# koadman/mauveAligner

Hardware: AMD Instinct MI355X
Metric: aligned Mbp/s (seed+extend+DP) (higher is better)
Workload: dtype u32

## Files before the change

mauvealigner_amd/csrc/chain_dev.hip:

```cpp
#include "common.hpp"
#include "dev_scan.hpp"
#include <cstring>
#include <cstdlib>

namespace {

using namespace devscan;
constexpr int CH_TILE = devscan::TILE;

constexpr int CH_CNT_ALIVE = 8, CH_CNT_CL = CH_CNT_ALIVE + MAUVE_MAX_SEQ, CH_CNT_WORDS = 128;
static_assert(CH_CNT_CL + MAUVE_MAX_SEQ <= CH_CNT_WORDS && CH_CNT_WORDS <= 256, "counter block");

struct ChKeyDst { uint32_t *key, *val, *key0, *val0; };
__device__ __forceinline__ void ch_put_key(const ChKeyDst &kd, uint32_t n, uint32_t i, int g, int32_t s, bool alive, uint32_t dead_key)
{
    uint32_t *k = g ? kd.key + (size_t)g * n : kd.key0, *v = g ? kd.val + (size_t)g * n : kd.val0;
    k[i] = alive ? (uint32_t)(s < 0 ? -s : s) : dead_key;
    v[i] = i;
}

__global__ void __launch_bounds__(256) ch_init(const int64_t *__restrict__ rlen, const int64_t *__restrict__ rst, uint32_t n, int N,
                                               int32_t *__restrict__ len, int32_t *__restrict__ st, uint32_t *__restrict__ crop,
                                               uint32_t *__restrict__ cnt, unsigned long long *__restrict__ weight, ChKeyDst kd, uint32_t dead_key)
{
// ... 116 lines not shown
    __device__ void total(uint32_t na, int y) const { if (y == 0) cnt[0] = na; }
};
struct LcbNodes {
    const int32_t *len, *st; uint32_t n; int N; const uint32_t *ordc, *rank; uint32_t *cnt; int32_t *node_of;
    unsigned long long *weight; uint32_t *orient; const uint32_t *gapid;
    const int64_t *mw;
    __device__ uint32_t domain(int) const { return cnt[0]; }
    __device__ bool flag(uint32_t k, int) const
    {
        if (k == 0) return true;
        const uint32_t i = ordc[k], p = ordc[k - 1];
        if (gapid && gapid[i] != gapid[p]) return true;
        bool brk = false;
#pragma unroll 4
        for (int g = 1; g < N; g++) {
            const bool oi = st[(size_t)i * N + g] < 0, op = st[(size_t)p * N + g] < 0;
            const uint32_t ri = rank[(size_t)g * n + i], rp = rank[(size_t)g * n + p];
            brk |= (oi != op) | (!oi ? ri != rp + 1 : ri + 1 != rp);
        }
        return brk;
    }
    __device__ void each(uint32_t k, uint32_t o, bool fl, int) const
    {
        const uint32_t i = ordc[k], nd = o + (fl ? 1u : 0u) - 1u;
        node_of[i] = (int32_t)nd;
        atomicAdd(&weight[nd], mw ? (unsigned long long)mw[i] : (unsigned long long)len[i] * (unsigned long long)N);
    }
    __device__ void emit(uint32_t k, uint32_t o, int) const
    {
        const uint32_t i = ordc[k];
        uint32_t ob = 0;
        for (int g = 0; g < N; g++) if (st[(size_t)i * N + g] < 0) ob |= 1u << g;
        orient[o] = ob;
    }
    __device__ void total(uint32_t K, int) const { cnt[1] = K; }
};
struct NodeSeq {
    uint32_t n; const uint32_t *ordc; uint32_t *cnt; const int32_t *node_of; int32_t *seq;
    __device__ uint32_t domain(int) const { return cnt[0]; }
    __device__ bool flag(uint32_t r, int y) const { return r == 0 || node_of[ordc[(size_t)y * n + r]] != node_of[ordc[(size_t)y * n + r - 1]]; }
    __device__ void each(uint32_t, uint32_t, bool, int) const {}
    __device__ void emit(uint32_t r, uint32_t o, int y) const { if (o < cnt[1]) seq[(size_t)y * cnt[1] + o] = node_of[ordc[(size_t)y * n + r]]; }
    __device__ void total(uint32_t t, int) const { if (t != cnt[1]) atomicAdd(&cnt[2], 1u); }
};
__global__ void __launch_bounds__(256) ch_links(int N, const uint32_t *__restrict__ cnt, const int32_t *__restrict__ seq,
                                                int32_t *__restrict__ prevv, int32_t *__restrict__ nextv)
{
    const uint32_t K = cnt[1], j = blockIdx.x * 256u + threadIdx.x;
    const int g = blockIdx.y;
// ... 85 lines not shown
        return;
    }
    uint32_t L[CH_CL_MAX], Ln[CH_CL_MAX], I[CH_CL_MAX], CF[CH_CL_MAX], CL[CH_CL_MAX], pf[CH_CL_MAX], pl[CH_CL_MAX];
    uint8_t F[CH_CL_MAX];
    ch_cluster_run(len, st, N, g, dead_key, eleft, eidx, a, s, L, Ln, I, CF, CL, pf, pl, F);
}

__global__ void __launch_bounds__(64) ch_cluster_pass_big(int32_t *__restrict__ len, int32_t *__restrict__ st, int N, int g, uint32_t dead_key,
                                                          uint32_t *__restrict__ eleft, uint32_t *__restrict__ eidx,
                                                          const uint32_t *__restrict__ cstart, const uint32_t *__restrict__ cnt_in,
                                                          uint32_t *__restrict__ ws, uint32_t n, int cl_max, uint32_t *__restrict__ fail, int big_max)
{
    const uint32_t j = blockIdx.x * 64u + threadIdx.x;
    if (j >= cnt_in[0]) return;
    const uint32_t a = cstart[j];
    const int s = (int)(cstart[j + 1] - a);
    if (s <= cl_max) return;
    if (s > big_max) { *fail = 1; return; }
    uint32_t *L = ws + a, *Ln = L + n, *I = Ln + n, *CF = I + n, *CL = CF + n, *pf = CL + n, *pl = pf + n;
    uint8_t *F = reinterpret_cast<uint8_t *>(ws + 7 * (size_t)n) + a;
    ch_cluster_run(len, st, N, g, dead_key, eleft, eidx, a, s, L, Ln, I, CF, CL, pf, pl, F);
}

__global__ void __launch_bounds__(256) ch_pack_graph(uint32_t K, int N, const unsigned long long *__restrict__ weight, const uint32_t *__restrict__ orient,
                                                     const int32_t *__restrict__ prevv, const int32_t *__restrict__ nextv, const uint32_t *__restrict__ cnt,
                                                     unsigned long long *__restrict__ out)
{
    const uint32_t i = blockIdx.x * 256u + threadIdx.x;
    uint32_t *o32 = reinterpret_cast<uint32_t *>(out + K);
    int32_t *op = reinterpret_cast<int32_t *>(o32 + K), *on = op + (size_t)K * N;
    if (i < K) { out[i] = weight[i]; o32[i] = orient[i]; }
    if (i < K * (uint32_t)N) { op[i] = prevv[i]; on[i] = nextv[i]; }
    if (i == 0) reinterpret_cast<uint32_t *>(on + (size_t)K * N)[0] = cnt[2];
}

__global__ void __launch_bounds__(256) ch_label(const int32_t *__restrict__ len, uint32_t n, const int32_t *__restrict__ node_of,
                                                const int32_t *__restrict__ final_id, int32_t *__restrict__ lcb)
{
    const uint32_t i = blockIdx.x * 256u + threadIdx.x;
    if (i >= n) return;
    lcb[i] = len[i] > 0 ? final_id[node_of[i]] : -1;
}

__global__ void __launch_bounds__(256) co_keys(const int32_t *__restrict__ lcb, const uint32_t *__restrict__ ord0, const uint32_t *__restrict__ cnt, uint32_t n, uint32_t nl,
                                               uint32_t *__restrict__ key, uint32_t *__restrict__ val, unsigned long long *__restrict__ lw, uint32_t *__restrict__ out)
{
    const uint32_t k = blockIdx.x * 256u + threadIdx.x;
    if (k < nl) lw[k] = 0;
    if (k < 2) out[k] = 0;
    if (k >= n) return;
    if (k < cnt[0]) {
// ... 117 lines not shown
        for (int j = lane; j < kk; j += 64) {
            int v = j;
            while (!s_alive[v] && s_merged[v] >= 0) v = s_merged[v];
            node_ok[n0 + j] = s_alive[v] ? 1 : 0;
        }
    }
}
struct GapSurvivors {
    const int32_t *len, *st, *node_of; const uint32_t *gapid; const uint8_t *node_ok; uint32_t n; int N;
    int32_t *olen, *ost; uint32_t *ogap; uint32_t *total_out;
    __device__ uint32_t domain(int) const { return n; }
    __device__ bool flag(uint32_t i, int) const { return len[i] > 0 && node_ok[node_of[i]]; }
    __device__ void each(uint32_t, uint32_t, bool, int) const {}
    __device__ void emit(uint32_t i, uint32_t o, int) const
    {
        olen[o] = len[i]; ogap[o] = gapid[i];
        for (int g = 0; g < N; g++) ost[(size_t)o * N + g] = st[(size_t)i * N + g];
    }
    __device__ void total(uint32_t t, int) const { *total_out = t; }
};

}

int chain_order_device(mauve_ctx *c, int N, int64_t nl, int64_t min_gap, int64_t *na_out, int64_t *n_rec_out)
{
    const uint32_t n = (uint32_t)c->dev_rec_n;
    *na_out = 0; *n_rec_out = 0;
    if (nl <= 0) return MAUVE_OK;
    const int32_t *len = c->ch_len.as<int32_t>(), *lcb = len + 2 * (size_t)n;
    const int32_t *st = c->ch_st.as<int32_t>();
    uint32_t *k1 = c->ch_ent.as<uint32_t>(), *v1 = k1 + n, *k2 = v1 + n, *v2 = k2 + n;
    HIPCHK(c, c->ch_anch.ensure((size_t)n * (2 + (size_t)N) * 4 + 64));
    HIPCHK(c, c->ch_lw.ensure((size_t)nl * 8 + 64));
    int32_t *alen = c->ch_anch.as<int32_t>(), *ast = alen + n, *alcb = ast + (size_t)n * N;
    unsigned long long *lw = c->ch_lw.as<unsigned long long>();
    uint32_t *cnt = c->ch_cnt.as<uint32_t>();
    const uint32_t blocks = (n + 255) / 256;
    int bits = 1; while ((1LL << bits) <= nl) bits++;
    hipLaunchKernelGGL(co_keys, dim3(blocks), dim3(256), 0, c->stream, lcb, c->ch_ord.as<uint32_t>() + (size_t)n * N , cnt, n, (uint32_t)nl, k1, v1, lw, cnt + 16);
    uint32_t *kk = k1, *vv = v1;
    int rc = sort_pairs_u32(c, n, bits, &kk, &vv, k2, v2, MAUVE_K_MISC);
    if (rc) return rc;
    hipLaunchKernelGGL(co_gather, dim3(blocks), dim3(256), 0, c->stream, kk, vv, n, (uint32_t)nl, N, len, st, min_gap, alen, ast, alcb, lw, cnt + 16);
    HIPCHK(c, hipGetLastError());
    HIPCHK(c, c->pin_chain.ensure(256));
    HIPCHK(c, hipMemcpyAsync(c->pin_chain.p, cnt + 16, 8, hipMemcpyDeviceToHost, c->stream));
    HIPCHK(c, hipStreamSynchronize(c->stream));
    *na_out = c->pin_chain.as<uint32_t>()[0];
    *n_rec_out = c->pin_chain.as<uint32_t>()[1];
    return MAUVE_OK;
}

struct ChSpGenomes { uint64_t word_off[MAUVE_MAX_SEQ]; int32_t s[4][4]; };
template <int MODE>
__global__ void __launch_bounds__(256) ch_sp_scores(const uint64_t *__restrict__ packed, ChSpGenomes G, int N, const int32_t *__restrict__ len, const int32_t *__restrict__ st,
                                                    uint32_t n, int64_t *__restrict__ out, SpMult M)
{
    const int lane = threadIdx.x & 63;
    const uint32_t wave = (blockIdx.x * 256u + threadIdx.x) >> 6, nw = (gridDim.x * 256u) >> 6;
    for (uint32_t i = wave; i < n; i += nw) {
        const int64_t L = len[i];
        int64_t acc = 0;
        for (int64_t c = lane; c < L; c += 64) {
            uint32_t have = 0, bases = 0;
            uint64_t mlo = 0, mhi = 0;
            for (int g = 0; g < N; g++) {
                const int64_t s0 = st[(size_t)i * N + g];
// ... 34 lines not shown
    HIPCHK(c, c->ch_st.ensure((size_t)n * N * 4));
    HIPCHK(c, c->ch_crop.ensure((size_t)n * 8));
    const uint32_t nb = (n + CH_TILE - 1) / CH_TILE;
    const size_t sl_words = ((size_t)N * ((size_t)n + 1) + 15) & ~(size_t)15, flag_bytes = ((size_t)N * n + 63) & ~(size_t)63;
    HIPCHK(c, c->ch_ent.ensure((size_t)n * 4 * 4 + sl_words * 4 + flag_bytes + (size_t)nb * 4 * 3 * (size_t)N + 64));
    HIPCHK(c, c->ch_ord.ensure((size_t)n * N * 4 * 3));
    HIPCHK(c, c->ch_rank.ensure((size_t)n * N * 4));
    HIPCHK(c, c->ch_cnt.ensure((size_t)CH_CNT_WORDS * 4));
    if (seg0) HIPCHK(c, c->ch_big.ensure((size_t)n * 29 + 64));
    int32_t *len = c->ch_len.as<int32_t>(), *node_of = len + n;
    uint32_t *gapid = seg0 ? reinterpret_cast<uint32_t *>(len + 3 * (size_t)n) : nullptr;
    int32_t *st = c->ch_st.as<int32_t>();
    uint32_t *crop = c->ch_crop.as<uint32_t>();
    uint32_t *sl = c->ch_ent.as<uint32_t>() + 4 * (size_t)n;
    uint8_t *cflag = reinterpret_cast<uint8_t *>(sl + sl_words);
    uint32_t *bmax = reinterpret_cast<uint32_t *>(cflag + flag_bytes), *balive = bmax + (size_t)N * nb, *bcnt = balive + (size_t)N * nb;
    uint32_t *ord = c->ch_ord.as<uint32_t>(), *ordc = ord + (size_t)n * N, *okey = ordc + (size_t)n * N;
    uint32_t *rank = c->ch_rank.as<uint32_t>();
    uint32_t *cnt = c->ch_cnt.as<uint32_t>();
    const int64_t *rlen = c->sorted_rec.as<int64_t>(), *rst = rlen + n;
    const uint32_t blocks = (n + 255) / 256;
    const int big_max = switches().ch_big_max;
    const int cl_set = switches().ch_cl_max, cl_max = cl_set && cl_set < CH_CL_MAX ? cl_set : CH_CL_MAX;
    HIPCHK(c, c->ch_graph.ensure((size_t)n * (8 + 4 + (size_t)N * 4 * 3 + 4) + 8 + (size_t)n * (8 + 4 + (size_t)N * 8) + 64));
    unsigned long long *weight = c->ch_graph.as<unsigned long long>();
    const int sort_passes = (pos_bits + 1 + 7) / 8;
    const bool odd = sort_passes & 1;
    const int g_lo = seg0 ? 0 : 1;
    const ChKeyDst kd{odd ? rank : okey, odd ? ordc : ord, seg0 && odd ? rank : okey, seg0 && odd ? ordc : ord};
    if (seg0) hipLaunchKernelGGL(ch_init_seg, dim3(blocks), dim3(256), 0, c->stream, rlen, rst, n, N, seg0, nseg, len, st, crop, gapid, cnt, weight, kd, dead_key);
    else hipLaunchKernelGGL(ch_init, dim3(blocks), dim3(256), 0, c->stream, rlen, rst, n, N, len, st, crop, cnt, weight, kd, dead_key);
    if (g_lo < N) {
        uint32_t *kk = kd.key + (size_t)g_lo * n, *vv = kd.val + (size_t)g_lo * n;
        int rc = sort_pairs_u32_batch(c, (uint32_t)(N - g_lo), n, n, pos_bits + 1, &kk, &vv, (odd ? okey : rank) + (size_t)g_lo * n,
                                      (odd ? ord : ordc) + (size_t)g_lo * n, MAUVE_K_MISC);
        if (rc) return rc;
        if (kk != okey + (size_t)g_lo * n || vv != ord + (size_t)g_lo * n) { c->err = "chain_device: the orders did not land in place"; return MAUVE_ERR_STATE; }
    }
    hipLaunchKernelGGL(cl_partial, dim3(nb, N), dim3(256), 0, c->stream, len, n, dead_key, okey, ord, bmax, balive);
    hipLaunchKernelGGL(cl_flags, dim3(nb, N), dim3(256), 0, c->stream, len, n, dead_key, okey, ord, bmax, balive, nb, cflag, cnt, bcnt);
    const ClusterStarts cs{cflag, n, sl, cnt};
    hipLaunchKernelGGL((cmp_write<ClusterStarts>), dim3(nb, N), dim3(256), 0, c->stream, cs, bcnt);
    for (int g = 0; g < N; g++) {
        uint32_t *og = ord + (size_t)g * n, *kg = okey + (size_t)g * n, *sg = sl + (size_t)g * ((size_t)n + 1);
        hipLaunchKernelGGL(ch_cluster_pass, dim3(blocks), dim3(256), 0, c->stream, len, st, N, g, dead_key, kg, og, sg, cnt + CH_CNT_CL + g, cnt + 3, seg0 ? 1 : 0, cl_max);
        if (seg0) hipLaunchKernelGGL(ch_cluster_pass_big, dim3((n + 63) / 64), dim3(64), 0, c->stream, len, st, N, g, dead_key, kg, og, sg, cnt + CH_CNT_CL + g,
                                     c->ch_big.as<uint32_t>(), n, cl_max, cnt + 3, big_max);
// ... 13 lines not shown
        memcpy(SG.s, sp_scoring->matrix, sizeof SG.s);
        SpMult M; memset(&M, 0, sizeof M);
        if (c->rp_now != MAUVE_REPEAT_PENALTY_OFF) {
            if (c->rp_gen != c->genome_gen) { c->err = "chain_device: repeat multiplicities missing"; return MAUVE_ERR_STATE; }
            M.p = c->rp_mult.as<uint8_t>();
            for (int g = 0; g < N; g++) M.off[g] = c->rp_off[(size_t)g];
        }
        const dim3 grid((uint32_t)std::min<size_t>(((size_t)n + 3) / 4, 256 * 8));
        if (c->rp_now == MAUVE_REPEAT_PENALTY_NEGATIVE)
            hipLaunchKernelGGL(ch_sp_scores<MAUVE_REPEAT_PENALTY_NEGATIVE>, grid, dim3(256), 0, c->stream, c->genomes.as<uint64_t>(), SG, N, len, st, n, c->ch_mw.as<int64_t>(), M);
        else if (c->rp_now == MAUVE_REPEAT_PENALTY_ZERO)
            hipLaunchKernelGGL(ch_sp_scores<MAUVE_REPEAT_PENALTY_ZERO>, grid, dim3(256), 0, c->stream, c->genomes.as<uint64_t>(), SG, N, len, st, n, c->ch_mw.as<int64_t>(), M);
        else
            hipLaunchKernelGGL(ch_sp_scores<MAUVE_REPEAT_PENALTY_OFF>, grid, dim3(256), 0, c->stream, c->genomes.as<uint64_t>(), SG, N, len, st, n, c->ch_mw.as<int64_t>(), M);
        mw = c->ch_mw.as<int64_t>();
    }
    const LcbNodes ln{len, st, n, N, ordc, rank, cnt, node_of, weight, orient, gapid, mw};
    hipLaunchKernelGGL((cmp_count<LcbNodes>), dim3(nb), dim3(256), 0, c->stream, ln, bcnt);
    hipLaunchKernelGGL((cmp_write<LcbNodes>), dim3(nb), dim3(256), 0, c->stream, ln, bcnt);
    const NodeSeq ns{n, ordc, cnt, node_of, seq};
    hipLaunchKernelGGL((cmp_count<NodeSeq>), dim3(nb, N), dim3(256), 0, c->stream, ns, bcnt);
    hipLaunchKernelGGL((cmp_write<NodeSeq>), dim3(nb, N), dim3(256), 0, c->stream, ns, bcnt);
    hipLaunchKernelGGL(ch_links, dim3(blocks, N), dim3(256), 0, c->stream, N, cnt, seq, prevv, nextv);
    HIPCHK(c, hipGetLastError());
    HIPCHK(c, c->pin_chain.ensure(256));
    HIPCHK(c, hipMemcpyAsync(c->pin_chain.p, cnt, 256, hipMemcpyDeviceToHost, c->stream));
    HIPCHK(c, hipStreamSynchronize(c->stream));
    const uint32_t *hc = c->pin_chain.as<uint32_t>();
    if (hc[3]) { c->err = "chain_device: overlap cluster beyond the per-thread limit"; return MAUVE_ERR_LIMIT; }
    const uint32_t na = hc[0], K = hc[1];
    G->na = na; G->K = K; G->weight = nullptr; G->orient = nullptr; G->prev = nullptr; G->next = nullptr; G->final_stage = nullptr; G->final_dev = final_dev;
    if (K && graph_to_host) {
        const size_t gbytes = (size_t)K * (8 + 4 + (size_t)N * 8) + 64;
        HIPCHK(c, c->pin_chain.ensure(256 + gbytes + (size_t)K * 4));
        char *pg = c->pin_chain.as<char>() + 256;
        int64_t *hw = reinterpret_cast<int64_t *>(pg);
        uint32_t *ho = reinterpret_cast<uint32_t *>(hw + K);
        int32_t *hp = reinterpret_cast<int32_t *>(ho + K), *hn = hp + (size_t)K * N;
        const size_t pbytes = (size_t)K * (8 + 4 + (size_t)N * 8) + 4;
        unsigned long long *pack = reinterpret_cast<unsigned long long *>((reinterpret_cast<uintptr_t>(final_dev + n) + 7) & ~(uintptr_t)7);
        hipLaunchKernelGGL(ch_pack_graph, dim3((K * (uint32_t)N + 255) / 256), dim3(256), 0, c->stream, K, N, weight, orient, prevv, nextv, cnt, pack);
        HIPCHK(c, hipMemcpyAsync(pg, pack, pbytes, hipMemcpyDeviceToHost, c->stream));
        HIPCHK(c, hipStreamSynchronize(c->stream));
        if (*reinterpret_cast<uint32_t *>(hn + (size_t)K * N)) { c->err = "chain_device: node lists inconsistent"; return MAUVE_ERR_LIMIT; }
        G->weight = hw; G->orient = ho; G->prev = hp; G->next = hn; G->final_stage = reinterpret_cast<int32_t *>(pg + gbytes);
    }
    if (trace) fprintf(stderr, "[trace] chain (device): eliminate+nodes+graph %.3f ms (na=%u K=%u)\n", now_ms() - t0, na, K);
    return MAUVE_OK;
}

int chain_device_core(mauve_ctx *c, int N, int64_t min_weight, bool collinear, int64_t &n_lcb, const mauve_scoring *sp_scoring)
{
    const bool trace = switches().trace;
    int64_t maxlen = 1; for (int g = 0; g < N; g++) maxlen = std::max<int64_t>(maxlen, c->lens[(size_t)g]);
    ChainGraphHost G;
    int rc = chain_device_graph(c, N, maxlen, nullptr, 0, &G, true, sp_scoring);
    if (rc) return rc;
    const double t1 = now_ms();
    const uint32_t n = (uint32_t)c->dev_rec_n, K = G.K, blocks = (n + 255) / 256;
    int32_t *len = c->ch_len.as<int32_t>(), *node_of = len + n, *lcb = node_of + n;
    n_lcb = 0;
    if (K) {
        std::vector<int64_t> final_id;
        lcb_greedy(N, (int32_t)K, G.weight, G.orient, G.prev, G.next, min_weight, collinear, final_id, n_lcb);
        for (uint32_t i = 0; i < K; i++) G.final_stage[i] = (int32_t)final_id[i];
        HIPCHK(c, hipMemcpyAsync(G.final_dev, G.final_stage, (size_t)K * 4, hipMemcpyHostToDevice, c->stream));
// ... 175 lines not shown
```

mauvealigner_amd/csrc/common.hpp:

```cpp
#pragma once
#include <hip/hip_runtime.h>
#include <cstdint>
#include <cstdio>
#include <string>
#include <vector>
#include <functional>
#include "switches.hpp"
#include "workers.hpp"
#include "host_chain.hpp"
#include "backbone_host.hpp"
#include <chrono>
#include <algorithm>
#include <cstring>

#include "../../include/mauve_hip.h"

#define HIPCHK(ctx, call)                                                                         \
    do {                                                                                          \
        hipError_t e__ = (call);                                                                  \
        if (e__ != hipSuccess) {                                                                  \
            (ctx)->err = std::string(#call) + ": " + hipGetErrorString(e__) + " (" __FILE__ ":" + \
                         std::to_string(__LINE__) + ")";                                          \
            return MAUVE_ERR_HIP;                                                                 \
        }                                                                                         \
// ... 373 lines not shown
    (void)hipStreamSynchronize(ctx->stream);
    const double t = now_ms();
    fprintf(stderr, "[trace] %-22s +%.3f ms\n", label, t - t0);
    t0 = t;
}
inline int seed_counters(mauve_ctx *ctx, size_t bytes, const uint32_t **words)
{
    HIPCHK(ctx, ctx->pin_seed.ensure(64));
    HIPCHK(ctx, hipMemcpyAsync(ctx->pin_seed.p, ctx->counters.p, bytes, hipMemcpyDeviceToHost, ctx->stream));
    HIPCHK(ctx, hipStreamSynchronize(ctx->stream));
    *words = ctx->pin_seed.as<uint32_t>();
    return MAUVE_OK;
}
int chain_device(mauve_ctx *c, int N, int64_t min_weight, bool collinear, MatchVec &m, std::vector<int64_t> &match_lcb, int64_t &n_lcb, const mauve_scoring *sp_scoring = nullptr);
struct ChainGraphHost { uint32_t na, K; int64_t *weight; uint32_t *orient; int32_t *prev, *next; int32_t *final_stage; int32_t *final_dev; };
int chain_device_graph(mauve_ctx *c, int N, int64_t maxlen, const uint32_t *seg0, uint32_t nseg, ChainGraphHost *G, bool graph_to_host = true, const mauve_scoring *sp_scoring = nullptr);
int chain_device_gaps_compact(mauve_ctx *c, int N, int64_t maxlen, const uint32_t *seg0_dev, uint32_t nseg, const int32_t **hl_out, const int32_t **hs_out,
                              const uint32_t **hgap_out, uint32_t *ns_out);
int chain_device_core(mauve_ctx *c, int N, int64_t min_weight, bool collinear, int64_t &n_lcb, const mauve_scoring *sp_scoring = nullptr);
int chain_device_gaps(mauve_ctx *c, int N, int64_t maxlen, const uint32_t *seg0_dev, uint32_t nseg, const int32_t **hl_out, const int32_t **hs_out,
                      const uint32_t **hgap_out, uint32_t *ns_out);
int recursive_anchoring(mauve_ctx *c, const mauve_params *p, int w0, std::vector<MatchVec> &chains, int N, const int *gmap);
int chain_device_copy_back(mauve_ctx *c, int N, MatchVec &m, std::vector<int64_t> &match_lcb);
int chain_order_device(mauve_ctx *c, int N, int64_t nl, int64_t min_gap, int64_t *na_out, int64_t *n_rec_out);
int extend_lcbs_device(mauve_ctx *c, const mauve_params *p, int w, int64_t lcbw, int N, const int32_t **alen_io, const int32_t **ast_io,
                       const int32_t **alcb_io, int64_t *na_io, int64_t *nl_io, int64_t *n_rec_io, std::vector<int64_t> &lcb_weight);

struct ChainOrders { std::vector<std::vector<uint32_t>> ord; bool sparse = false; };
void host_eliminate_overlaps(MatchVec &m, ChainOrders *orders = nullptr, bool compact = true);
int seed_family_matches(mauve_ctx *c, const GenomeSet &gs, int w, int mode, uint64_t mask, MatchVec &out);
void host_merge_matches(MatchVec &kept, const MatchVec &add);
void host_left_orders(const MatchVec &m, ChainOrders &orders);
void host_lcb_chain(const MatchVec &m, int64_t min_weight, bool collinear, std::vector<int64_t> &match_lcb, int64_t &n_lcb,
                    const ChainOrders *orders = nullptr, const int64_t *match_weight = nullptr);
int match_sp_scores(mauve_ctx *c, const MatchVec &m, const int *gmap, const mauve_scoring *sc, std::vector<int64_t> &out);
int repeat_multiplicity(mauve_ctx *c, uint64_t pattern);
int repeat_matches(mauve_ctx *c, int seq, uint64_t pattern, int64_t min_multi, int64_t max_multi);
int repeat_fetch(mauve_ctx *c, int64_t *length, int64_t *mult, int64_t *start_off, int64_t *starts);
int repeat_begin(mauve_ctx *c, const mauve_params *p, int w, uint64_t pat);
int64_t sp_default_min_weight(int w, int n, const mauve_scoring *sc);
int resolve_seed(mauve_ctx *c, const mauve_params *p, int64_t avg_len, const char *who, int *w, uint64_t *pat);
void seed_matches_to_vec(const mauve_ctx *c, int n, int64_t nm, MatchVec &m);
int host_chain_lcbs(mauve_ctx *c, const mauve_params *p, MatchVec &m, const int *gmap, int64_t lcbw, int64_t minw_sp, std::vector<int64_t> &match_lcb,
                    int64_t &nl, std::vector<int64_t> *match_weight, bool compact, double *t_elim = nullptr);
void result_reset(AlignResult &R);
void restore_cols(AlignResult &R, uint32_t full, SpinPool *pool = nullptr);

// ... 52 lines not shown
```

mauvealigner_amd/csrc/dev_scan.hpp:

```cpp
#pragma once
#include <hip/hip_runtime.h>
#include <cstdint>

namespace devscan {

constexpr int TILE = 1024;

__device__ __forceinline__ uint32_t bscan_add(uint32_t v, uint32_t *total, uint32_t *lds )
{
    const int lane = threadIdx.x & 63, wave = threadIdx.x >> 6;
    uint32_t inc = v;
#pragma unroll
    for (int o = 1; o < 64; o <<= 1) { const uint32_t t = __shfl_up(inc, o); if (lane >= o) inc += t; }
    __syncthreads();
    if (lane == 63) lds[wave] = inc;
    __syncthreads();
    uint32_t wbase = 0, tot = 0;
#pragma unroll
    for (int w = 0; w < 4; w++) { const uint32_t c = lds[w]; if (w < wave) wbase += c; tot += c; }
    *total = tot;
    return wbase + inc - v;
}
__device__ __forceinline__ uint32_t bscan_max(uint32_t v, uint32_t *total, uint32_t *lds )
{
// ... 14 lines not shown
__device__ __forceinline__ void tiles_before_add(const uint32_t *__restrict__ v, uint32_t b, uint32_t nb, uint32_t *before, uint32_t *all, uint32_t *lds)
{
    uint32_t sb = 0, sa = 0;
    for (uint32_t t = threadIdx.x; t < nb; t += 256) { const uint32_t x = v[t]; sa += x; if (t < b) sb += x; }
    uint32_t tb, ta;
    (void)bscan_add(sb, &tb, lds); (void)bscan_add(sa, &ta, lds);
    *before = tb; *all = ta;
}

__device__ __forceinline__ void wave_keyed_add(unsigned long long *arr, bool active, uint32_t l, unsigned long long v)
{
    const uint64_t act = __ballot(active);
    if (!act) return;
    const int first = __ffsll((unsigned long long)act) - 1;
    const uint32_t l0 = (uint32_t)__shfl((int)l, first);
    if (__ballot(active && l == l0) == act) {
        unsigned long long s = active ? v : 0ull;
#pragma unroll
        for (int o = 32; o > 0; o >>= 1) s += __shfl_xor(s, o);
        if ((int)(threadIdx.x & 63) == first) atomicAdd(&arr[l0], s);
    } else if (active) atomicAdd(&arr[l], v);
}

template <class F>
__global__ void __launch_bounds__(256) cmp_count(F f, uint32_t *__restrict__ bcnt)
{
    __shared__ uint32_t lds[4];
    const int y = blockIdx.y;
    const uint32_t dom = f.domain(y), r0 = blockIdx.x * (uint32_t)TILE + threadIdx.x * 4u;
    uint32_t c = 0;
#pragma unroll
    for (int i = 0; i < 4; i++) if (r0 + i < dom) c += f.flag(r0 + i, y) ? 1u : 0u;
    uint32_t tc;
    (void)bscan_add(c, &tc, lds);
    if (threadIdx.x == 0) bcnt[(size_t)y * gridDim.x + blockIdx.x] = tc;
}
template <class F>
__global__ void __launch_bounds__(256) cmp_write(F f, const uint32_t *__restrict__ bcnt)
{
    __shared__ uint32_t lds[4];
    const int y = blockIdx.y;
    const uint32_t dom = f.domain(y), r0 = blockIdx.x * (uint32_t)TILE + threadIdx.x * 4u;
    uint32_t before, all;
    tiles_before_add(bcnt + (size_t)y * gridDim.x, blockIdx.x, gridDim.x, &before, &all, lds);
    bool fl[4]; uint32_t c = 0;
#pragma unroll
    for (int i = 0; i < 4; i++) { fl[i] = r0 + i < dom && f.flag(r0 + i, y); c += fl[i] ? 1u : 0u; }
    uint32_t dummy;
    uint32_t o = before + bscan_add(c, &dummy, lds);
#pragma unroll
    for (int i = 0; i < 4; i++) {
        if (r0 + i >= dom) break;
        f.each(r0 + i, o, fl[i], y);
        if (fl[i]) { f.emit(r0 + i, o, y); o++; }
    }
    if (blockIdx.x == 0 && threadIdx.x == 0) f.total(all, y);
}


template <class T, class In>
__global__ void __launch_bounds__(256) vscan_partial(In in, uint32_t n, T *__restrict__ bsum)
{
    __shared__ T red[4];
    const uint32_t r0 = blockIdx.x * (uint32_t)TILE + threadIdx.x * 4u;
    T s = 0;
#pragma unroll
    for (int i = 0; i < 4; i++) if (r0 + i < n) s += in.value(r0 + i);
#pragma unroll
    for (int o = 32; o > 0; o >>= 1) s += __shfl_down(s, o);
    if ((threadIdx.x & 63) == 0) red[threadIdx.x >> 6] = s;
    __syncthreads();
    if (threadIdx.x == 0) bsum[blockIdx.x] = red[0] + red[1] + red[2] + red[3];
}
template <class T, class In>
__global__ void __launch_bounds__(256) vscan_write(In in, uint32_t n, const T *__restrict__ bsum, T *__restrict__ out, T *__restrict__ total)
{
    __shared__ T red[4];
    __shared__ T s_before, s_all;
// ... 75 lines not shown
```

mauvealigner_amd/csrc/extend_dev.hip:

```cpp
#include "common.hpp"
#include <algorithm>
#include <cstdlib>
#include <cstring>

namespace {

__global__ void __launch_bounds__(256) ext_lcb_ends(const int32_t *__restrict__ alcb, uint32_t na, uint32_t *__restrict__ first_a, uint32_t *__restrict__ last_a)
{
    const uint32_t a = blockIdx.x * 256u + threadIdx.x;
    if (a >= na) return;
    const int32_t l = alcb[a];
    if (a == 0 || alcb[a - 1] != l) first_a[l] = a;
    if (a + 1 == na || alcb[a + 1] != l) last_a[l] = a;
}

__global__ void __launch_bounds__(256) ext_lcb_extents(const int32_t *__restrict__ alen, const int32_t *__restrict__ ast, int N, uint32_t nl,
                                                       const uint32_t *__restrict__ first_a, const uint32_t *__restrict__ last_a,
                                                       int64_t *__restrict__ left, int64_t *__restrict__ right)
{
    const uint32_t t = blockIdx.x * 256u + threadIdx.x;
    if (t >= nl * (uint32_t)N) return;
    const uint32_t l = t / (uint32_t)N; const int g = (int)(t % (uint32_t)N);
    const uint32_t a0 = first_a[l], a1 = last_a[l];
    const int64_t s0 = ast[(size_t)a0 * N + g], s1 = ast[(size_t)a1 * N + g];
    int64_t le, re;
    if (s0 > 0) { le = s0; re = s1 + alen[a1] - 1; }
    else { le = -s1; re = -s0 + alen[a0] - 1; }
    left[t] = s0 < 0 ? -le : le; right[t] = s0 < 0 ? -re : re;
}

struct ExtGatherArgs { uint64_t src_word_off[MAUVE_MAX_SEQ], dst_word_off[MAUVE_MAX_SEQ], dst_words[MAUVE_MAX_SEQ]; };
__device__ __forceinline__ uint64_t spread_bits32(uint32_t x)
{
    uint64_t v = x;
    v = (v | (v << 16)) & 0x0000ffff0000ffffULL; v = (v | (v << 8)) & 0x00ff00ff00ff00ffULL; v = (v | (v << 4)) & 0x0f0f0f0f0f0f0f0fULL;
    v = (v | (v << 2)) & 0x3333333333333333ULL; v = (v | (v << 1)) & 0x5555555555555555ULL;
    return v;
}
__global__ void __launch_bounds__(256) ext_gather(const uint64_t *__restrict__ genomes, uint64_t *__restrict__ out, ExtGatherArgs ga,
                                                  const uint32_t *__restrict__ vs, const int64_t *__restrict__ rs, const uint32_t *__restrict__ ln, uint32_t K)
{
    const int g = blockIdx.y;
    const uint64_t p = (uint64_t)blockIdx.x * 256 + threadIdx.x;
    const uint64_t w0 = p >> 5 & ~(uint64_t)1;
    if (w0 >= ga.dst_words[g]) return;
    const uint32_t *v = vs + (size_t)g * (K + 1);
// ... 69 lines not shown
            mx = max(mx, hi - lo + 1);
        }
        f = mx > min_gap;
    }
    flag[j] = f;
}

struct LcbTab {
    int N = 0; int64_t n = 0;
    std::vector<int64_t> lo, hi, weight;
    std::vector<uint32_t> rev;
};

}

int rec_gap_flags_device(mauve_ctx *c, const int32_t *alen, const int32_t *ast, const int32_t *alcb, int64_t na, int N, int64_t min_gap, uint8_t *d_flag)
{
    if (na <= 0) return MAUVE_OK;
    hipLaunchKernelGGL(ext_flag_rec, dim3((uint32_t)((na + 255) / 256)), dim3(256), 0, c->stream, alen, ast, alcb, (uint32_t)na, N, min_gap, d_flag);
    HIPCHK(c, hipGetLastError());
    return MAUVE_OK;
}

int extend_lcbs_device(mauve_ctx *c, const mauve_params *p, int w, int64_t lcbw, int N, const int32_t **alen_io, const int32_t **ast_io,
                       const int32_t **alcb_io, int64_t *na_io, int64_t *nl_io, int64_t *n_rec_io, std::vector<int64_t> &lcb_weight)
{
    const bool trace = switches().trace;
    const double t0 = now_ms();
    const uint32_t na = (uint32_t)*na_io; const int64_t nl0 = *nl_io;
    const int32_t *alen = *alen_io, *ast = *ast_io, *alcb = *alcb_io;
    const uint32_t full = full_mask(N);
    LcbTab T; T.N = N; T.n = nl0;
    {
        const size_t o_last = (size_t)nl0 * 4, o_left = (o_last + (size_t)nl0 * 4 + 7) & ~(size_t)7, o_right = o_left + (size_t)nl0 * N * 8, total = o_right + (size_t)nl0 * N * 8;
        HIPCHK(c, c->ext_work.ensure(total + 64));
        char *wk = c->ext_work.as<char>();
        uint32_t *first_a = reinterpret_cast<uint32_t *>(wk), *last_a = reinterpret_cast<uint32_t *>(wk + o_last);
        int64_t *left = reinterpret_cast<int64_t *>(wk + o_left), *right = reinterpret_cast<int64_t *>(wk + o_right);
        hipLaunchKernelGGL(ext_lcb_ends, dim3((na + 255) / 256), dim3(256), 0, c->stream, alcb, na, first_a, last_a);
        hipLaunchKernelGGL(ext_lcb_extents, dim3(((uint32_t)nl0 * N + 255) / 256), dim3(256), 0, c->stream, alen, ast, N, (uint32_t)nl0, first_a, last_a, left, right);
        HIPCHK(c, hipGetLastError());
        const size_t eb = 2 * (size_t)nl0 * N * 8;
        HIPCHK(c, c->pin_ext.ensure(eb + (size_t)nl0 * 8 + 64));
        HIPCHK(c, hipMemcpyAsync(c->pin_ext.p, left, eb, hipMemcpyDeviceToHost, c->stream));
        HIPCHK(c, hipMemcpyAsync(c->pin_ext.as<char>() + eb, c->ch_lw.p, (size_t)nl0 * 8, hipMemcpyDeviceToHost, c->stream));
        HIPCHK(c, hipStreamSynchronize(c->stream));
        const int64_t *hl = c->pin_ext.as<int64_t>(), *hr = hl + (size_t)nl0 * N, *hw = hr + (size_t)nl0 * N;
        T.lo.resize((size_t)nl0 * N); T.hi.resize((size_t)nl0 * N); T.weight.assign(hw, hw + nl0); T.rev.assign((size_t)nl0, 0u);
        for (int64_t l = 0; l < nl0; l++)
            for (int g = 0; g < N; g++) {
                const int64_t a = hl[(size_t)l * N + g], b = hr[(size_t)l * N + g];
                T.lo[(size_t)l * N + g] = std::llabs(a); T.hi[(size_t)l * N + g] = std::llabs(b);
                if (a < 0) T.rev[(size_t)l] |= 1u << g;
            }
    }
    const bool keep_pending = c->matches_pending; const int64_t keep_n = c->n_matches, keep_rec = c->dev_rec_n; const int keep_nseq = c->match_nseq;
    std::swap(c->sorted_rec, c->sorted_rec_keep);
    auto restore = [&]() {
        std::swap(c->sorted_rec, c->sorted_rec_keep);
        c->matches_pending = keep_pending; c->n_matches = keep_n; c->dev_rec_n = keep_rec; c->match_nseq = keep_nseq;
        if (keep_pending) { c->match_len.clear(); c->match_start.clear(); }
    };
    MatchVec added(N); std::vector<int64_t> added_lcb;
    std::vector<int64_t> cur_of_orig((size_t)nl0);
    for (int64_t l = 0; l < nl0; l++) cur_of_orig[(size_t)l] = l;
    int w_e = w;
    for (int iter = 0; iter < p->max_extension_iters; iter++) {
        w_e -= 2;
        if (w_e < 5) break;
// ... 166 lines not shown
```

mauvealigner_amd/csrc/pipeline.cpp:

```cpp
#include "common.hpp"
#include <algorithm>
#include <cstdlib>
#include <cstring>

namespace {

inline uint8_t base_at(const uint64_t *w, int64_t i) { return (uint8_t)((w[(size_t)(i >> 5)] >> (2 * (i & 31))) & 3); }

}

static int extend_lcbs(mauve_ctx *c, const mauve_params *p, int w, int64_t lcbw, MatchVec &m, std::vector<int64_t> &match_lcb,
                       int64_t &nl)
{
    const int N = m.N;
    const uint32_t full = full_mask(N);
    int w_e = w;
    MatchVec base(N); ChainOrders base_ord; bool have_base = false;
    for (int iter = 0; iter < p->max_extension_iters; iter++) {
        w_e -= 2;
        if (w_e < 5) break;
        const uint64_t pe = mauve_get_seed(w_e, 0);
        if (!pe) break;
        const int64_t span_e = mauve_seed_length(pe);
        const bool trace = switches().trace;
// ... 244 lines not shown
        rc = seedpass_run(c, main_genome_set(c), pat, p->mode, full, 1, nullptr, 0, &nm);
        c->lazy_matches_ok = false;
        c->shadow = nullptr;
        if (rc) return rc;
    }
    S.nm = nm;
    if (!c->matches_pending) { R.mum_length = c->match_len; R.mum_start = c->match_start; }
    const double t1 = now_ms();
    c->stage.seed_ms = t1 - S.t0;

    MatchVec &m = S.m; m.N = N;
    const int64_t lcbw = p->lcb_weight >= 0 ? p->lcb_weight : (int64_t)3 * w * N;
    std::vector<int64_t> &match_lcb = S.match_lcb; int64_t nl = 0;
    if (p->lcb_scoring != MAUVE_LCB_SCORE_LENGTH && p->lcb_scoring != MAUVE_LCB_SCORE_SP) { c->err = "align: unknown lcb_scoring"; return MAUVE_ERR_ARG; }
    bool on_device = !switches().host_chain && nm > 0 && c->dev_rec_n == nm && p->lcb_scoring == MAUVE_LCB_SCORE_LENGTH;
    double t1b = t1;
    if (on_device) {
        rc = chain_device_core(c, N, lcbw, p->collinear != 0, nl);
        if (rc == MAUVE_ERR_LIMIT) on_device = false;
        else if (rc) return rc;
        else {
            if (want_tail && !switches().host_tail && (!do_extend || ext_on_device) && nl > 0) {
                int64_t na = 0, nrec = 0;
                rc = chain_order_device(c, N, nl, p->min_recursive_gap, &na, &nrec);
                if (rc) return rc;
                const uint32_t cap = (uint32_t)c->dev_rec_n;
                S.dv_len = c->ch_anch.as<int32_t>(); S.dv_st = S.dv_len + cap; S.dv_lcb = S.dv_st + (size_t)cap * N;
                bool ext_declined = false;
                if (do_extend && na >= 1) {
                    std::vector<int64_t> lw;
                    rc = extend_lcbs_device(c, p, w, lcbw, N, &S.dv_len, &S.dv_st, &S.dv_lcb, &na, &nl, &nrec, lw);
                    if (rc == MAUVE_ERR_LIMIT) { ext_declined = true; rc = MAUVE_OK; c->err.clear(); }
                    else if (rc) return rc;
                    else { R.lcb_weight.swap(lw); S.lw_from_host = true; }
                }
                if (ext_declined) { S.dv_len = S.dv_st = S.dv_lcb = nullptr; }
                else if (na >= 2 && (!p->recursive || nrec == 0)) {
                    S.nl = nl; S.n_anchor = na; S.dev_tail = true;
                    if (c->pf.live) HIPCHK(c, hipEventRecord(c->ev_io_fork, c->stream));
                    const double t2 = now_ms();
                    c->stage.chain_ms = t2 - t1;
                    if (switches().trace) fprintf(stderr, "[trace] chain: on the device %.3f ms, %lld anchors in %lld LCBs stay there\n", t2 - t1, (long long)na, (long long)nl);
                    S.t_dp0 = t2;
                    S.open = true;
                    return MAUVE_OK;
                }
                if (do_extend && !ext_declined) {
// ... 710 lines not shown
```

Measured before the change: 11100.

## Cut host syncs in device chaining and aggregate per-node weight atomics

Node weights are now summed per thread across runs of equal node ids, and across the wave with a segmented shuffle scan, so fewer 64-bit atomics hit the same node. The graph pack kernel is launched before the first sync and copies the counter block plus a 128KB prefix of the graph in one transfer, so small graphs need only a single round trip. The LCB extent table kernels and their copies are queued inside chain_order_device, before its existing sync, using the device-side anchor count. That removes a separate stream synchronization in the extension step. The cost is more complex scan code and a pack kernel sized to n rather than K.

```diff
diff --git a/mauvealigner_amd/csrc/chain_dev.hip b/mauvealigner_amd/csrc/chain_dev.hip
--- a/mauvealigner_amd/csrc/chain_dev.hip
+++ b/mauvealigner_amd/csrc/chain_dev.hip
@@ -162,9 +162,26 @@
     }
     __device__ void each(uint32_t k, uint32_t o, bool fl, int) const
     {
-        const uint32_t i = ordc[k], nd = o + (fl ? 1u : 0u) - 1u;
-        node_of[i] = (int32_t)nd;
-        atomicAdd(&weight[nd], mw ? (unsigned long long)mw[i] : (unsigned long long)len[i] * (unsigned long long)N);
+        node_of[ordc[k]] = (int32_t)(o + (fl ? 1u : 0u) - 1u);
+    }
+    __device__ void quad(uint32_t k0, uint32_t o, const bool *fl, int cnt_in, int) const
+    {
+        uint32_t nd0 = 0, nd = 0; unsigned long long hs = 0, s = 0;
+#pragma unroll
+        for (int q = 0; q < 4; q++) {
+            if (q >= cnt_in) break;
+            const uint32_t i = ordc[k0 + q];
+            const unsigned long long v = mw ? (unsigned long long)mw[i] : (unsigned long long)len[i] * (unsigned long long)N;
+            o += fl[q] ? 1u : 0u;
+            const uint32_t x = o - 1u;
+            if (q == 0) { nd0 = nd = x; s = v; }
+            else if (x == nd) s += v;
+            else {
+                if (nd == nd0) hs = s; else atomicAdd(&weight[nd], s);
+                nd = x; s = v;
+            }
+        }
+        wave_runs_add(weight, cnt_in > 0, nd0, hs, nd, s);
     }
     __device__ void emit(uint32_t k, uint32_t o, int) const
     {
@@ -296,11 +313,16 @@
     ch_cluster_run(len, st, N, g, dead_key, eleft, eidx, a, s, L, Ln, I, CF, CL, pf, pl, F);
 }
 
-__global__ void __launch_bounds__(256) ch_pack_graph(uint32_t K, int N, const unsigned long long *__restrict__ weight, const uint32_t *__restrict__ orient,
+constexpr size_t CH_CNT_BYTES = 256;
+static_assert(CH_CNT_BYTES <= (size_t)CH_CNT_WORDS * 4 && CH_CNT_BYTES % 8 == 0, "the host's part of the counter block");
+constexpr size_t CH_PACK_PREFIX = 128 << 10;
+__global__ void __launch_bounds__(256) ch_pack_graph(int N, const unsigned long long *__restrict__ weight, const uint32_t *__restrict__ orient,
                                                      const int32_t *__restrict__ prevv, const int32_t *__restrict__ nextv, const uint32_t *__restrict__ cnt,
                                                      unsigned long long *__restrict__ out)
 {
-    const uint32_t i = blockIdx.x * 256u + threadIdx.x;
+    const uint32_t K = cnt[1], i = blockIdx.x * 256u + threadIdx.x;
+    if (i < CH_CNT_BYTES / 4) reinterpret_cast<uint32_t *>(out)[i] = cnt[i];
+    out += CH_CNT_BYTES / 8;
     uint32_t *o32 = reinterpret_cast<uint32_t *>(out + K);
     int32_t *op = reinterpret_cast<int32_t *>(o32 + K), *on = op + (size_t)K * N;
     if (i < K) { out[i] = weight[i]; o32[i] = orient[i]; }
@@ -464,7 +486,7 @@
 
 }
 
-int chain_order_device(mauve_ctx *c, int N, int64_t nl, int64_t min_gap, int64_t *na_out, int64_t *n_rec_out)
+int chain_order_device(mauve_ctx *c, int N, int64_t nl, int64_t min_gap, int64_t *na_out, int64_t *n_rec_out, bool ext_table)
 {
     const uint32_t n = (uint32_t)c->dev_rec_n;
     *na_out = 0; *n_rec_out = 0;
@@ -485,6 +507,7 @@
     if (rc) return rc;
     hipLaunchKernelGGL(co_gather, dim3(blocks), dim3(256), 0, c->stream, kk, vv, n, (uint32_t)nl, N, len, st, min_gap, alen, ast, alcb, lw, cnt + 16);
     HIPCHK(c, hipGetLastError());
+    if (ext_table) { rc = extend_lcb_table_queue(c, N, nl, alen, ast, alcb, n, cnt + 16); if (rc) return rc; }
     HIPCHK(c, c->pin_chain.ensure(256));
     HIPCHK(c, hipMemcpyAsync(c->pin_chain.p, cnt + 16, 8, hipMemcpyDeviceToHost, c->stream));
     HIPCHK(c, hipStreamSynchronize(c->stream));
@@ -565,7 +588,7 @@
     const uint32_t blocks = (n + 255) / 256;
     const int big_max = switches().ch_big_max;
     const int cl_set = switches().ch_cl_max, cl_max = cl_set && cl_set < CH_CL_MAX ? cl_set : CH_CL_MAX;
-    HIPCHK(c, c->ch_graph.ensure((size_t)n * (8 + 4 + (size_t)N * 4 * 3 + 4) + 8 + (size_t)n * (8 + 4 + (size_t)N * 8) + 64));
+    HIPCHK(c, c->ch_graph.ensure((size_t)n * (8 + 4 + (size_t)N * 4 * 3 + 4) + 8 + CH_CNT_BYTES + (size_t)n * (8 + 4 + (size_t)N * 8) + 64));
     unsigned long long *weight = c->ch_graph.as<unsigned long long>();
     const int sort_passes = (pos_bits + 1 + 7) / 8;
     const bool odd = sort_passes & 1;
@@ -625,26 +648,38 @@
     hipLaunchKernelGGL((cmp_count<NodeSeq>), dim3(nb, N), dim3(256), 0, c->stream, ns, bcnt);
     hipLaunchKernelGGL((cmp_write<NodeSeq>), dim3(nb, N), dim3(256), 0, c->stream, ns, bcnt);
     hipLaunchKernelGGL(ch_links, dim3(blocks, N), dim3(256), 0, c->stream, N, cnt, seq, prevv, nextv);
-    HIPCHK(c, hipGetLastError());
-    HIPCHK(c, c->pin_chain.ensure(256));
-    HIPCHK(c, hipMemcpyAsync(c->pin_chain.p, cnt, 256, hipMemcpyDeviceToHost, c->stream));
+    const size_t node_bytes = 8 + 4 + (size_t)N * 8;
+    const size_t pack_cap = CH_CNT_BYTES + (size_t)n * node_bytes + 4;
+    const size_t head = graph_to_host ? std::min(CH_PACK_PREFIX, pack_cap) : CH_CNT_BYTES;
+    HIPCHK(c, c->pin_chain.ensure(head + 64 + head / node_bytes * 4 + 64));
+    if (graph_to_host) {
+        unsigned long long *pack = reinterpret_cast<unsigned long long *>((reinterpret_cast<uintptr_t>(final_dev + n) + 7) & ~(uintptr_t)7);
+        hipLaunchKernelGGL(ch_pack_graph, dim3((uint32_t)(((size_t)n * N + 255) / 256)), dim3(256), 0, c->stream, N, weight, orient, prevv, nextv, cnt, pack);
+        HIPCHK(c, hipGetLastError());
+        HIPCHK(c, hipMemcpyAsync(c->pin_chain.p, pack, head, hipMemcpyDeviceToHost, c->stream));
+    } else {
+        HIPCHK(c, hipGetLastError());
+        HIPCHK(c, hipMemcpyAsync(c->pin_chain.p, cnt, CH_CNT_BYTES, hipMemcpyDeviceToHost, c->stream));
+    }
     HIPCHK(c, hipStreamSynchronize(c->stream));
     const uint32_t *hc = c->pin_chain.as<uint32_t>();
     if (hc[3]) { c->err = "chain_device: overlap cluster beyond the per-thread limit"; return MAUVE_ERR_LIMIT; }
     const uint32_t na = hc[0], K = hc[1];
     G->na = na; G->K = K; G->weight = nullptr; G->orient = nullptr; G->prev = nullptr; G->next = nullptr; G->final_stage = nullptr; G->final_dev = final_dev;
     if (K && graph_to_host) {
-        const size_t gbytes = (size_t)K * (8 + 4 + (size_t)N * 8) + 64;
-        HIPCHK(c, c->pin_chain.ensure(256 + gbytes + (size_t)K * 4));
-        char *pg = c->pin_chain.as<char>() + 256;
+        const size_t gbytes = (size_t)K * node_bytes + 64, pbytes = (size_t)K * node_bytes + 4;
+        if (CH_CNT_BYTES + pbytes > head) {
+            const unsigned long long *pack = reinterpret_cast<const unsigned long long *>((reinterpret_cast<uintptr_t>(final_dev + n) + 7) & ~(uintptr_t)7);
+            const void *was = c->pin_chain.p;
+            HIPCHK(c, c->pin_chain.ensure(CH_CNT_BYTES + gbytes + (size_t)K * 4));
+            const size_t from = c->pin_chain.p == was ? head : CH_CNT_BYTES;
+            HIPCHK(c, hipMemcpyAsync(c->pin_chain.as<char>() + from, reinterpret_cast<const char *>(pack) + from, CH_CNT_BYTES + pbytes - from, hipMemcpyDeviceToHost, c->stream));
+            HIPCHK(c, hipStreamSynchronize(c->stream));
+        }
+        char *pg = c->pin_chain.as<char>() + CH_CNT_BYTES;
         int64_t *hw = reinterpret_cast<int64_t *>(pg);
         uint32_t *ho = reinterpret_cast<uint32_t *>(hw + K);
         int32_t *hp = reinterpret_cast<int32_t *>(ho + K), *hn = hp + (size_t)K * N;
-        const size_t pbytes = (size_t)K * (8 + 4 + (size_t)N * 8) + 4;
-        unsigned long long *pack = reinterpret_cast<unsigned long long *>((reinterpret_cast<uintptr_t>(final_dev + n) + 7) & ~(uintptr_t)7);
-        hipLaunchKernelGGL(ch_pack_graph, dim3((K * (uint32_t)N + 255) / 256), dim3(256), 0, c->stream, K, N, weight, orient, prevv, nextv, cnt, pack);
-        HIPCHK(c, hipMemcpyAsync(pg, pack, pbytes, hipMemcpyDeviceToHost, c->stream));
-        HIPCHK(c, hipStreamSynchronize(c->stream));
         if (*reinterpret_cast<uint32_t *>(hn + (size_t)K * N)) { c->err = "chain_device: node lists inconsistent"; return MAUVE_ERR_LIMIT; }
         G->weight = hw; G->orient = ho; G->prev = hp; G->next = hn; G->final_stage = reinterpret_cast<int32_t *>(pg + gbytes);
     }
diff --git a/mauvealigner_amd/csrc/common.hpp b/mauvealigner_amd/csrc/common.hpp
--- a/mauvealigner_amd/csrc/common.hpp
+++ b/mauvealigner_amd/csrc/common.hpp
@@ -419,7 +419,8 @@
                       const uint32_t **hgap_out, uint32_t *ns_out);
 int recursive_anchoring(mauve_ctx *c, const mauve_params *p, int w0, std::vector<MatchVec> &chains, int N, const int *gmap);
 int chain_device_copy_back(mauve_ctx *c, int N, MatchVec &m, std::vector<int64_t> &match_lcb);
-int chain_order_device(mauve_ctx *c, int N, int64_t nl, int64_t min_gap, int64_t *na_out, int64_t *n_rec_out);
+int chain_order_device(mauve_ctx *c, int N, int64_t nl, int64_t min_gap, int64_t *na_out, int64_t *n_rec_out, bool ext_table = false);
+int extend_lcb_table_queue(mauve_ctx *c, int N, int64_t nl, const int32_t *alen, const int32_t *ast, const int32_t *alcb, uint32_t cap, const uint32_t *na_dev);
 int extend_lcbs_device(mauve_ctx *c, const mauve_params *p, int w, int64_t lcbw, int N, const int32_t **alen_io, const int32_t **ast_io,
                        const int32_t **alcb_io, int64_t *na_io, int64_t *nl_io, int64_t *n_rec_io, std::vector<int64_t> &lcb_weight);
 
diff --git a/mauvealigner_amd/csrc/dev_scan.hpp b/mauvealigner_amd/csrc/dev_scan.hpp
--- a/mauvealigner_amd/csrc/dev_scan.hpp
+++ b/mauvealigner_amd/csrc/dev_scan.hpp
@@ -60,6 +60,33 @@
     } else if (active) atomicAdd(&arr[l], v);
 }
 
+__device__ __forceinline__ void wave_runs_add(unsigned long long *arr, bool has, uint32_t k0, unsigned long long hs, uint32_t kt, unsigned long long ts)
+{
+    const int lane = threadIdx.x & 63;
+    const bool split = has && k0 != kt;
+    const uint32_t kt_prev = (uint32_t)__shfl_up((int)kt, 1);
+    int f = (!has || split || lane == 0 || kt_prev != kt) ? 1 : 0;
+    unsigned long long s = has ? ts : 0ull;
+#pragma unroll
+    for (int o = 1; o < 64; o <<= 1) {
+        const unsigned long long t = __shfl_up(s, o);
+        const int g = __shfl_up(f, o);
+        if (lane >= o) { if (!f) s += t; f |= g; }
+    }
+    const unsigned long long s_prev = __shfl_up(s, 1);
+    const uint32_t k0_next = (uint32_t)__shfl_down((int)k0, 1);
+    const bool has_next = __shfl_down(has ? 1 : 0, 1) != 0 && lane < 63;
+    if (split) atomicAdd(&arr[k0], hs + (lane > 0 && kt_prev == k0 ? s_prev : 0ull));
+    if (has && !(has_next && k0_next == kt)) atomicAdd(&arr[kt], s);
+}
+
+template <class F>
+__device__ __forceinline__ auto cmp_quad(const F &f, uint32_t r0, uint32_t o0, const bool *fl, int cnt, int y, int) -> decltype(f.quad(r0, o0, fl, cnt, y))
+{
+    f.quad(r0, o0, fl, cnt, y);
+}
+template <class F>
+__device__ __forceinline__ void cmp_quad(const F &, uint32_t, uint32_t, const bool *, int, int, long) {}
 template <class F>
 __global__ void __launch_bounds__(256) cmp_count(F f, uint32_t *__restrict__ bcnt)
 {
@@ -85,13 +112,15 @@
 #pragma unroll
     for (int i = 0; i < 4; i++) { fl[i] = r0 + i < dom && f.flag(r0 + i, y); c += fl[i] ? 1u : 0u; }
     uint32_t dummy;
-    uint32_t o = before + bscan_add(c, &dummy, lds);
+    const uint32_t o0 = before + bscan_add(c, &dummy, lds);
+    uint32_t o = o0;
 #pragma unroll
     for (int i = 0; i < 4; i++) {
         if (r0 + i >= dom) break;
         f.each(r0 + i, o, fl[i], y);
         if (fl[i]) { f.emit(r0 + i, o, y); o++; }
     }
+    cmp_quad(f, r0, o0, fl, r0 >= dom ? 0 : (int)min(4u, dom - r0), y, 0);
     if (blockIdx.x == 0 && threadIdx.x == 0) f.total(all, y);
 }
 
diff --git a/mauvealigner_amd/csrc/extend_dev.hip b/mauvealigner_amd/csrc/extend_dev.hip
--- a/mauvealigner_amd/csrc/extend_dev.hip
+++ b/mauvealigner_amd/csrc/extend_dev.hip
@@ -5,9 +5,9 @@
 
 namespace {
 
-__global__ void __launch_bounds__(256) ext_lcb_ends(const int32_t *__restrict__ alcb, uint32_t na, uint32_t *__restrict__ first_a, uint32_t *__restrict__ last_a)
-{
-    const uint32_t a = blockIdx.x * 256u + threadIdx.x;
+__global__ void __launch_bounds__(256) ext_lcb_ends(const int32_t *__restrict__ alcb, const uint32_t *__restrict__ na_p, uint32_t *__restrict__ first_a, uint32_t *__restrict__ last_a)
+{
+    const uint32_t a = blockIdx.x * 256u + threadIdx.x, na = *na_p;
     if (a >= na) return;
     const int32_t l = alcb[a];
     if (a == 0 || alcb[a - 1] != l) first_a[l] = a;
@@ -15,13 +15,14 @@
 }
 
 __global__ void __launch_bounds__(256) ext_lcb_extents(const int32_t *__restrict__ alen, const int32_t *__restrict__ ast, int N, uint32_t nl,
-                                                       const uint32_t *__restrict__ first_a, const uint32_t *__restrict__ last_a,
+                                                       const uint32_t *__restrict__ first_a, const uint32_t *__restrict__ last_a, const uint32_t *__restrict__ na_p,
                                                        int64_t *__restrict__ left, int64_t *__restrict__ right)
 {
     const uint32_t t = blockIdx.x * 256u + threadIdx.x;
     if (t >= nl * (uint32_t)N) return;
     const uint32_t l = t / (uint32_t)N; const int g = (int)(t % (uint32_t)N);
-    const uint32_t a0 = first_a[l], a1 = last_a[l];
+    const uint32_t a0 = first_a[l], a1 = last_a[l], na = *na_p;
+    if (a0 >= na || a1 >= na) return;
     const int64_t s0 = ast[(size_t)a0 * N + g], s1 = ast[(size_t)a1 * N + g];
     int64_t le, re;
     if (s0 > 0) { le = s0; re = s1 + alen[a1] - 1; }
@@ -137,6 +138,23 @@
     return MAUVE_OK;
 }
 
+int extend_lcb_table_queue(mauve_ctx *c, int N, int64_t nl, const int32_t *alen, const int32_t *ast, const int32_t *alcb, uint32_t cap, const uint32_t *na_dev)
+{
+    const size_t o_last = (size_t)nl * 4, o_left = (o_last + (size_t)nl * 4 + 7) & ~(size_t)7, o_right = o_left + (size_t)nl * N * 8, total = o_right + (size_t)nl * N * 8;
+    HIPCHK(c, c->ext_work.ensure(total + 64));
+    char *wk = c->ext_work.as<char>();
+    uint32_t *first_a = reinterpret_cast<uint32_t *>(wk), *last_a = reinterpret_cast<uint32_t *>(wk + o_last);
+    int64_t *left = reinterpret_cast<int64_t *>(wk + o_left), *right = reinterpret_cast<int64_t *>(wk + o_right);
+    hipLaunchKernelGGL(ext_lcb_ends, dim3((cap + 255) / 256), dim3(256), 0, c->stream, alcb, na_dev, first_a, last_a);
+    hipLaunchKernelGGL(ext_lcb_extents, dim3(((uint32_t)nl * N + 255) / 256), dim3(256), 0, c->stream, alen, ast, N, (uint32_t)nl, first_a, last_a, na_dev, left, right);
+    HIPCHK(c, hipGetLastError());
+    const size_t eb = 2 * (size_t)nl * N * 8;
+    HIPCHK(c, c->pin_ext.ensure(eb + (size_t)nl * 8 + 64));
+    HIPCHK(c, hipMemcpyAsync(c->pin_ext.p, left, eb, hipMemcpyDeviceToHost, c->stream));
+    HIPCHK(c, hipMemcpyAsync(c->pin_ext.as<char>() + eb, c->ch_lw.p, (size_t)nl * 8, hipMemcpyDeviceToHost, c->stream));
+    return MAUVE_OK;
+}
+
 int extend_lcbs_device(mauve_ctx *c, const mauve_params *p, int w, int64_t lcbw, int N, const int32_t **alen_io, const int32_t **ast_io,
                        const int32_t **alcb_io, int64_t *na_io, int64_t *nl_io, int64_t *n_rec_io, std::vector<int64_t> &lcb_weight)
 {
@@ -147,19 +165,6 @@
     const uint32_t full = full_mask(N);
     LcbTab T; T.N = N; T.n = nl0;
     {
-        const size_t o_last = (size_t)nl0 * 4, o_left = (o_last + (size_t)nl0 * 4 + 7) & ~(size_t)7, o_right = o_left + (size_t)nl0 * N * 8, total = o_right + (size_t)nl0 * N * 8;
-        HIPCHK(c, c->ext_work.ensure(total + 64));
-        char *wk = c->ext_work.as<char>();
-        uint32_t *first_a = reinterpret_cast<uint32_t *>(wk), *last_a = reinterpret_cast<uint32_t *>(wk + o_last);
-        int64_t *left = reinterpret_cast<int64_t *>(wk + o_left), *right = reinterpret_cast<int64_t *>(wk + o_right);
-        hipLaunchKernelGGL(ext_lcb_ends, dim3((na + 255) / 256), dim3(256), 0, c->stream, alcb, na, first_a, last_a);
-        hipLaunchKernelGGL(ext_lcb_extents, dim3(((uint32_t)nl0 * N + 255) / 256), dim3(256), 0, c->stream, alen, ast, N, (uint32_t)nl0, first_a, last_a, left, right);
-        HIPCHK(c, hipGetLastError());
-        const size_t eb = 2 * (size_t)nl0 * N * 8;
-        HIPCHK(c, c->pin_ext.ensure(eb + (size_t)nl0 * 8 + 64));
-        HIPCHK(c, hipMemcpyAsync(c->pin_ext.p, left, eb, hipMemcpyDeviceToHost, c->stream));
-        HIPCHK(c, hipMemcpyAsync(c->pin_ext.as<char>() + eb, c->ch_lw.p, (size_t)nl0 * 8, hipMemcpyDeviceToHost, c->stream));
-        HIPCHK(c, hipStreamSynchronize(c->stream));
         const int64_t *hl = c->pin_ext.as<int64_t>(), *hr = hl + (size_t)nl0 * N, *hw = hr + (size_t)nl0 * N;
         T.lo.resize((size_t)nl0 * N); T.hi.resize((size_t)nl0 * N); T.weight.assign(hw, hw + nl0); T.rev.assign((size_t)nl0, 0u);
         for (int64_t l = 0; l < nl0; l++)
diff --git a/mauvealigner_amd/csrc/pipeline.cpp b/mauvealigner_amd/csrc/pipeline.cpp
--- a/mauvealigner_amd/csrc/pipeline.cpp
+++ b/mauvealigner_amd/csrc/pipeline.cpp
@@ -290,7 +290,7 @@
         else {
             if (want_tail && !switches().host_tail && (!do_extend || ext_on_device) && nl > 0) {
                 int64_t na = 0, nrec = 0;
-                rc = chain_order_device(c, N, nl, p->min_recursive_gap, &na, &nrec);
+                rc = chain_order_device(c, N, nl, p->min_recursive_gap, &na, &nrec, do_extend);
                 if (rc) return rc;
                 const uint32_t cap = (uint32_t)c->dev_rec_n;
                 S.dv_len = c->ch_anch.as<int32_t>(); S.dv_st = S.dv_len + cap; S.dv_lcb = S.dv_st + (size_t)cap * N;
```

New measurement: 11010. About the same (-0.9%).
